# lukasvst/dm-vio

Measured on NVIDIA H100. Metric: point-residuals/sec per GN iter (7 KF, 2000 pts, 640x480), higher is better.
Workload: dtype f32

## Files before the change

### dm-vio_b200/csrc/ba_fused.cu

```cuda
#include "ba_common.cuh"
#include <cstdlib>
#include <mutex>
#include <type_traits>

namespace dmv {

template <int K, int END, class F>
__device__ __forceinline__ void static_for(F&& f) {
  if constexpr (K < END) {
    f(std::integral_constant<int, K>{});
    static_for<K + 1, END>(f);
  }
}
__host__ __device__ constexpr int top_row(int k) {
  int r = 0;
  while (r < 9 && k >= top_off(r + 1)) r++;
  return r;
}
__host__ __device__ constexpr int top_col(int k) { return top_row(k) + k - top_off(top_row(k)); }

struct PixSums {
  float JI00, JI10, JI11, JabJI00, JabJI01, JabJI10, JabJI11, Jab00, Jab01, Jab11, JIr0, JIr1, Jabr0, Jabr1, rr;
};

// ... 591 lines not shown
        const float gx = h1 * hw, gy = h2 * hw;
        const float resF = residual * hw;
        const float ja = drdA * hw, jb = hw;
        const float jaF = zA ? 0.f : ja, jbF = zB ? 0.f : jb;
        float ra = resF;
        if constexpr (MARG) { ra = (((resF - gx * jpx) - gy * jpy) - jaF * dp6) - jbF * dp7; rtz[jj] = ra; }
        sv[0] += gx * gx; sv[2] += gy * gy; sv[1] += gx * gy;
        sv[3] += ja * gx; sv[4] += ja * gy; sv[5] += jb * gx; sv[6] += jb * gy;
        sv[7] += ja * ja; sv[8] += ja * jb; sv[9] += jb * jb;
        sv[10] += ra * gx; sv[11] += ra * gy; sv[12] += ra * jaF; sv[13] += ra * jbF; sv[14] += ra * ra;
        sv[16] += hw * hw * (gx * gx + gy * gy);
      }
    }
    clk_stamp<CLK>(clk, 3, __float_as_uint(sv[0]));
    {
      const unsigned bal = __ballot_sync(0xffffffffu, fin);
      live = live && (((bal >> (lane & ~3)) & 0xfu) == 0xfu);
#pragma unroll
      for (int k = 0; k < 17; k++) {
        sv[k] += __shfl_xor_sync(0xffffffffu, sv[k], 1);
        sv[k] += __shfl_xor_sync(0xffffffffu, sv[k], 2);
      }
    }
    PixSums s = {sv[0], sv[1], sv[2], sv[3], sv[4], sv[5], sv[6], sv[7], sv[8], sv[9], sv[10], sv[11], sv[12], sv[13], sv[14]};
    const float energy = sv[15], wJI2 = sv[16];

    int newState;
    float newEnergy;
    if (st == RES_NONE) { newState = RES_NONE; newEnergy = 0.f; }
    else if (!live) { newState = RES_OOB; newEnergy = en_old; }
    else if (energy > TH || wJI2 < 2.f) { newState = RES_OUTLIER; newEnergy = TH; }
    else { newState = RES_IN; newEnergy = energy; }
    const bool in = (newState == RES_IN);
    if (st != RES_NONE && q == 0) {
      e_sum = newEnergy;
      n_in = in; n_oob = (newState == RES_OOB); n_outl = (newState == RES_OUTLIER);
    }
    if constexpr (MARG) {
      if (masked) *reinterpret_cast<float2*>(W.marg_rtz + (size_t)slot * 8 + 2 * q) = in ? make_float2(rtz[0], rtz[1]) : make_float2(0.f, 0.f);
    }
    if (valid && masked && q == 0) {
      W.st_new[slot] = (uint8_t)newState;
      W.en_new[slot] = newEnergy;
      const float ewo = (st == RES_NONE || !live) ? -1.f : energy;
      W.en_wo[slot] = ewo;
      if (t == nf - 1 && W.en_wo_newest_host) W.en_wo_newest_host[p] = ewo;
      const size_t plane = (size_t)MAXF * mp;
      W.cpt[slot] = cKu; W.cpt[plane + slot] = cKv; W.cpt[2 * plane + slot] = new_idepth;
    }

    float jp[8] = {0.f, 0.f, 0.f, 0.f, 0.f, 0.f, 0.f, 0.f}, Hdd = 0.f, bd = 0.f, Hcd0 = 0.f, Hcd1 = 0.f, Hcd2 = 0.f, Hcd3 = 0.f;
    if (in) {
      if constexpr (!MARG) geo_jac(pc, Kl0, Kl1, cu, cv, drescale, new_idepth, fx, fy, fxi, fyi, x, y, ddx, ddy);
      const float J0 = s.JI00 * ddx + s.JI10 * ddy, J1 = s.JI10 * ddx + s.JI11 * ddy;
#pragma unroll
      for (int k = 0; k < 6; k++) jp[k] = x[4 + k] * J0 + y[4 + k] * J1;
      jp[6] = s.JabJI00 * ddx + s.JabJI01 * ddy; jp[7] = s.JabJI10 * ddx + s.JabJI11 * ddy;
      Hdd = J0 * ddx + J1 * ddy;
      bd = s.JIr0 * ddx + s.JIr1 * ddy;
      Hcd0 = x[0] * J0 + y[0] * J1; Hcd1 = x[1] * J0 + y[1] * J1; Hcd2 = x[2] * J0 + y[2] * J1; Hcd3 = x[3] * J0 + y[3] * J1;
      if (valid && q == 0) {
        float4* gj = reinterpret_cast<float4*>(W.jpjd + (size_t)slot * 8);
        gj[0] = make_float4(jp[0], jp[1], jp[2], jp[3]);
        gj[1] = make_float4(jp[4], jp[5], jp[6], jp[7]);
      }
    } else {
#pragma unroll
      for (int k = 0; k < 10; k++) { x[k] = 0.f; y[k] = 0.f; }
      s = PixSums{0.f, 0.f, 0.f, 0.f, 0.f, 0.f, 0.f, 0.f, 0.f, 0.f, 0.f, 0.f, 0.f, 0.f, 0.f};
    }
    {
      const float r0 = ah[0].x * jp[0] + ah[0].y * jp[1] + ah[0].z * jp[2] + ah[0].w * jp[3] + ah[1].x * jp[4] + ah[1].y * jp[5] + ah[1].z * jp[6] + ah[1].w * jp[7];
      const float r1 = ah[2].x * jp[0] + ah[2].y * jp[1] + ah[2].z * jp[2] + ah[2].w * jp[3] + ah[3].x * jp[4] + ah[3].y * jp[5] + ah[3].z * jp[6] + ah[3].w * jp[7];
      const float j0 = (q == 0) ? jp[0] : (q == 1) ? jp[2] : (q == 2) ? jp[4] : jp[6];
      const float j1 = (q == 0) ? jp[1] : (q == 1) ? jp[3] : (q == 2) ? jp[5] : jp[7];
      if (pair_ok) {
        S.rec[t][2 * q][pl] = r0; S.rec[t][2 * q + 1][pl] = r1;
        S.Wv[pl][4 + 8 * t + 2 * q] = at2.x * j0; S.Wv[pl][4 + 8 * t + 2 * q + 1] = at2.y * j1;
      }
      const float e0 = (q == 0) ? Hdd : (q == 1) ? Hcd0 : (q == 2) ? Hcd2 : (in ? 1.f : 0.f);
      const float e1 = (q == 0) ? bd : (q == 1) ? Hcd1 : (q == 2) ? Hcd3 : 0.f;
      const int k0 = (q == 0) ? 8 : (q == 1) ? 10 : (q == 2) ? 12 : 14;
      if (pair_ok) { S.rec[t][k0][pl] = e0; S.rec[t][k0 + 1][pl] = e1; }
    }

    float v[32];
    {
      const float alq[3] = {s.JI00 * ((q == 0) ? x[0] : (q == 1) ? x[1] : (q == 2) ? x[2] : x[3]) + s.JI10 * ((q == 0) ? y[0] : (q == 1) ? y[1] : (q == 2) ? y[2] : y[3]),
                            s.JI00 * ((q == 0) ? x[4] : (q == 1) ? x[5] : (q == 2) ? x[6] : x[7]) + s.JI10 * ((q == 0) ? y[4] : (q == 1) ? y[5] : (q == 2) ? y[6] : y[7]),
                            s.JI00 * ((q == 0) ? x[8] : (q == 1) ? x[9] : 0.f) + s.JI10 * ((q == 0) ? y[8] : (q == 1) ? y[9] : 0.f)};
      const float beq[3] = {s.JI10 * ((q == 0) ? x[0] : (q == 1) ? x[1] : (q == 2) ? x[2] : x[3]) + s.JI11 * ((q == 0) ? y[0] : (q == 1) ? y[1] : (q == 2) ? y[2] : y[3]),
                            s.JI10 * ((q == 0) ? x[4] : (q == 1) ? x[5] : (q == 2) ? x[6] : x[7]) + s.JI11 * ((q == 0) ? y[4] : (q == 1) ? y[5] : (q == 2) ? y[6] : y[7]),
                            s.JI10 * ((q == 0) ? x[8] : (q == 1) ? x[9] : 0.f) + s.JI11 * ((q == 0) ? y[8] : (q == 1) ? y[9] : 0.f)};
      const float xq[3] = {(q == 0) ? x[0] : (q == 1) ? x[1] : (q == 2) ? x[2] : x[3], (q == 0) ? x[4] : (q == 1) ? x[5] : (q == 2) ? x[6] : x[7],
                           (q == 0) ? x[8] : (q == 1) ? x[9] : 0.f};
      const float yq[3] = {(q == 0) ? y[0] : (q == 1) ? y[1] : (q == 2) ? y[2] : y[3], (q == 0) ? y[4] : (q == 1) ? y[5] : (q == 2) ? y[6] : y[7],
                           (q == 0) ? y[8] : (q == 1) ? y[9] : 0.f};
      int o = 0;
#pragma unroll
      for (int j = 0; j < 3; j++) {
#pragma unroll
        for (int c = 4 * j; c < 13; c++) {
          float val;
          if (c < 10) val = alq[j] * x[c] + beq[j] * y[c];
          else if (c == 10) val = xq[j] * s.JabJI00 + yq[j] * s.JabJI01;
          else if (c == 11) val = xq[j] * s.JabJI10 + yq[j] * s.JabJI11;
          else val = xq[j] * s.JIr0 + yq[j] * s.JIr1;
          v[o++] = val;
        }
      }
      if (q == 2) { v[22] = s.Jab00; v[23] = s.Jab01; v[24] = s.Jabr0; v[25] = s.Jab11; v[26] = s.Jabr1; }
      v[27] = (q == 2) ? s.rr : 0.f;
      if (q == 3) { v[22] = v[23] = v[24] = v[25] = v[26] = 0.f; }
      v[28] = v[29] = v[30] = v[31] = 0.f;
    }
    static_for<0, 3>([&](auto sc) {
      constexpr int st2 = decltype(sc)::value, hstep = 16 >> st2, m = 16 >> st2;
      const bool up = (lane & m) != 0;
#pragma unroll
      for (int k = 0; k < hstep; k++) v[k] = (up ? v[k + hstep] : v[k]) + __shfl_xor_sync(0xffffffffu, up ? v[k] : v[k + hstep], m);
    });
    if (pair_ok) {
      const int w8 = (lane >> 2) & 7;
#pragma unroll
      for (int k = 0; k < 4; k++) {
        const int pos = 4 * w8 + k;
        int idx = -1;
        if (pos < 13) { const int rr = q, c = pos; if (c >= rr) idx = top_off(rr) + c - rr; }
        else if (pos < 22) { const int rr = q + 4, c = pos - 13 + 4; if (c >= rr) idx = top_off(rr) + c - rr; }
        else if (pos < 28) {
          if (q < 2) { const int rr = q + 8, c = pos - 22 + 8; if (pos < 27 && c >= rr) idx = top_off(rr) + c - rr; }
          else if (q == 2) idx = TOP_TRI + (pos - 22);
        }
        if (idx >= 0) S.pair[t][half][idx] = v[k];
      }
    }
  }
  }
  {
    float es = e_sum, fin = (float)n_in, foob = (float)n_oob, fout = (float)n_outl;
#pragma unroll
    for (int m = 1; m < 32; m <<= 1) {
      es += __shfl_xor_sync(0xffffffffu, es, m);
      fin += __shfl_xor_sync(0xffffffffu, fin, m);
      foob += __shfl_xor_sync(0xffffffffu, foob, m);
      fout += __shfl_xor_sync(0xffffffffu, fout, m);
      rs_step2 += __shfl_xor_sync(0xffffffffu, rs_step2, m);
      rs_nid += __shfl_xor_sync(0xffffffffu, rs_nid, m);
      rs_cnt += __shfl_xor_sync(0xffffffffu, rs_cnt, m);
    }
    if (lane == 0) {
      S.misc[warp][0] = es; S.misc[warp][1] = fin; S.misc[warp][2] = foob; S.misc[warp][3] = fout;
      S.misc[warp][4] = rs_step2; S.misc[warp][5] = rs_nid; S.misc[warp][6] = rs_cnt; S.misc[warp][7] = 0.f;
    }
  }
  cp_async_wait_all();
  __syncthreads();
  clk_stamp<CLK>(clk, 4);

  const int nt = nf - 1;
  double* __restrict__ out = W.part + (size_t)chunk * PART_STRIDE;
  {
    const int nG = nt * 26;
#pragma unroll 1
    for (int e = tid; e < nG + 9 * P + 28; e += nthreads) {
      if (e < nG) {
        const int rh = e / 13, c = e - rh * 13, i0 = (rh & 1) * 4;
        const int t = (rh >> 1) + ((rh >> 1) >= h ? 1 : 0);
        const int col = (c < 8) ? 4 + c : (c < 12 ? c - 8 : 12);
        double m[8];
#pragma unroll
        for (int k = 0; k < 8; k++) m[k] = (double)pair_entry<NH>(S.pair[t], 4 + k, col);
        const double dTc = S.dT[t][c & 7];
        const int os = (c < 8) ? 8 : (c < 12 ? 4 : 1);
        double* o = out + t * PART_SLOT + ((c < 8) ? 64 + c : (c < 12 ? 120 + c : 160)) + i0 * os;
#pragma unroll
        for (int ii = 0; ii < 4; ii++) {
          const int i = i0 + ii;
          double g = 0.0;
#pragma unroll
          for (int k = 0; k < 8; k++) g += S.AhD[t][i * 8 + k] * m[k];
          S.G[t][i][c] = g;
          double v = S.dT[t][i] * (i0 ? m[4 + ii] : m[ii]);
          if (c < 8) v = v * dTc;
          o[ii * os] = v;
        }
      } else if (e < nG + 9 * P) {
        const int k = (e - nG) / P, pl2 = (e - nG) & (P - 1);
        if (pl2 >= ch_count) continue;
        if (k < 8) {
          float sum = 0.f;
#pragma unroll
          for (int tt = 0; tt < MAXF; tt++) {
            const float v = S.rec[tt][k][pl2];
            if (tt < nf && tt != h) sum += v;
          }
          S.Wv[pl2][4 + 8 * h + k] = sum;
        } else {
          const int p = ch_start + pl2;
          float Hdd = 0.f, bd = 0.f, c0 = 0.f, c1 = 0.f, c2 = 0.f, c3 = 0.f, ngood = 0.f;
#pragma unroll 1
          for (int r = 0; r < nt; r++) {
            const int tt = r + (r >= h ? 1 : 0);
            Hdd += S.rec[tt][8][pl2]; bd += S.rec[tt][9][pl2]; c0 += S.rec[tt][10][pl2]; c1 += S.rec[tt][11][pl2];
            c2 += S.rec[tt][12][pl2]; c3 += S.rec[tt][13][pl2]; ngood += S.rec[tt][14][pl2];
          }
          float prior = S.prior[pl2];
          bool masked = true;
          if constexpr (MARG) { masked = __ldg(W.marg_mask + p) != 0; prior *= __ldg(&W.marg->priorFac); }
          float HdiF = 0.f, bdSum = 0.f, w0 = 0.f, w1 = 0.f, w2 = 0.f, w3 = 0.f;
          if (ngood > 0.f) {
            float H = Hdd + prior;
            if (H < 1e-10f) H = 1e-10f;
            HdiF = 1.0f / H;
            bdSum = MARG ? bd : bd + prior * (S.id[pl2] - S.idz[pl2]);
            w0 = c0; w1 = c1; w2 = c2; w3 = c3;
          }
          S.Wv[pl2][0] = w0; S.Wv[pl2][1] = w1; S.Wv[pl2][2] = w2; S.Wv[pl2][3] = w3;
          S.Wv[pl2][N] = bdSum;
#pragma unroll 1
          for (int c = N + 1; c < W.NW; c++) S.Wv[pl2][c] = 0.f;
          S.hdi[pl2] = HdiF;
          if (masked) {
            float4* po = reinterpret_cast<float4*>(W.pout + (size_t)p * 8);
            po[0] = make_float4(Hdd, bd, c0, c1);
            po[1] = make_float4(c2, c3, HdiF, bdSum);
          }
        }
      } else if (e < nG + 9 * P + 20) {
        const int i = (e - nG - 9 * P) / 5, j = (e - nG - 9 * P) - i * 5;
        double val = 0.0;
#pragma unroll 1
        for (int r = 0; r < nt; r++) val += (double)pair_entry<NH>(S.pair[r + (r >= h ? 1 : 0)], i, j < 4 ? j : 12);
        out[PART_CC + (j < 4 ? i * 4 + j : 16 + i)] = val;
      } else {
        const int k = e - nG - 9 * P - 20;
        double val = 0.0;
#pragma unroll 1
        for (int wv = 0; wv < nwarps; wv += 4) {
          float v[4];
#pragma unroll
          for (int u = 0; u < 4; u++) v[u] = S.misc[min(wv + u, 15)][k];
#pragma unroll
          for (int u = 0; u < 4; u++)
            if (wv + u < nwarps) val += (double)v[u];
        }
        out[PART_MISC + k] = val;
      }
    }
  }
  __syncthreads();
  {
    const int nO = nt * 16;
#pragma unroll 1
    for (int e = tid; e < 64 + nO + 8 + P * W.T; e += nthreads) {
      if (e < 64) {
        const int i = e >> 3, j = e & 7;
        double val = 0.0;
        double2 g[4], a[4];
        const int t0 = (h == 0) ? 1 : 0;
#pragma unroll
        for (int u = 0; u < 4; u++) { g[u] = reinterpret_cast<const double2*>(&S.G[t0][i][0])[u]; a[u] = reinterpret_cast<const double2*>(&S.AhD[t0][j * 8])[u]; }
#pragma unroll 1
        for (int r = 0; r < nt; r++) {
          const int tn = min(r + 1 + (r + 1 >= h ? 1 : 0), MAXF - 1);
          double2 gn[4], an[4];
#pragma unroll
          for (int u = 0; u < 4; u++) { gn[u] = reinterpret_cast<const double2*>(&S.G[tn][i][0])[u]; an[u] = reinterpret_cast<const double2*>(&S.AhD[tn][j * 8])[u]; }
#pragma unroll
          for (int u = 0; u < 4; u++) { val += g[u].x * a[u].x; val += g[u].y * a[u].y; }
#pragma unroll
          for (int u = 0; u < 4; u++) { g[u] = gn[u]; a[u] = an[u]; }
        }
        out[h * PART_SLOT + 64 + e] = val;
      } else if (e < 64 + nO) {
        const int eo = e - 64, r = eo >> 4, i = (eo >> 1) & 7, j0 = (eo & 1) * 4;
        const int t = r + (r >= h ? 1 : 0);
#pragma unroll
        for (int v = 0; v < 4; v++) out[t * PART_SLOT + i * 8 + j0 + v] = S.G[t][i][j0 + v] * S.dT[t][j0 + v];
      } else if (e < 64 + nO + 8) {
        const int i = e - 64 - nO;
        double c0 = 0.0, c1 = 0.0, c2 = 0.0, c3 = 0.0, bh = 0.0;
#pragma unroll 1
        for (int r = 0; r < nt; r++) {
          const int t2 = r + (r >= h ? 1 : 0);
          const double2 q01 = *reinterpret_cast<const double2*>(&S.G[t2][i][8]), q23 = *reinterpret_cast<const double2*>(&S.G[t2][i][10]);
          c0 += q01.x; c1 += q01.y; c2 += q23.x; c3 += q23.y; bh += S.G[t2][i][12];
        }
        double* o = out + h * PART_SLOT;
        o[128 + i * 4] = c0; o[128 + i * 4 + 1] = c1; o[128 + i * 4 + 2] = c2; o[128 + i * 4 + 3] = c3;
        o[160 + i] = bh;
      } else {
        const int ew = e - 64 - nO - 8, g4 = ew / P, pl2 = ew & (P - 1);
        if (pl2 >= ch_count) continue;
        W.wg[(size_t)g4 * mp + ch_start + pl2] = *reinterpret_cast<const float4*>(&S.Wv[pl2][4 * g4]);
        if (g4 == 0) W.hdig[ch_start + pl2] = S.hdi[pl2];
      }
    }
  }
  __syncthreads();
  clk_stamp<CLK>(clk, 5);
}

template <int P, int LPR, bool CLK = false>
__device__ __forceinline__ void fused_reduce(const BAWinDev& W, FusedSmem<P, LPR>& S, bool ok, const int vcta, const int ncta,
                                             unsigned long long* clk = nullptr) {
  const int nf = W.nf, N = W.N, mp = W.mp;
  const int tid = threadIdx.x, nthreads = blockDim.x;
  const int warp = tid >> 5, lane = tid & 31, nwarps = nthreads >> 5;

  const int nH = N * N + N;
  double* __restrict__ R = W.result;
  double* __restrict__ RH = W.result_host;
  const bool xch = W.xc.nranks > 1;
  const double* __restrict__ part = W.part;

  const int npair = nf * (nf - 1) / 2;
  const int n_off = npair * 64, n_diag = nf * 64, n_c = nf * 32, n_b = nf * 8;
  const int nitems = n_off + n_diag + n_c + n_b + 16 + 4 + (ACC_MISC - 1);
  const int grp = tid >> 4, gl = tid & 15, groups_per_cta = nthreads >> 4;
  const int nch = W.nchunks;
  const int dcta = ncta - 1 - vcta;
  auto phase_d = [&](const int pass) {
    for (int base = dcta * groups_per_cta; base < nitems; base += ncta * groups_per_cta) {
      const int item = base + grp;
      const bool act = item < nitems;
      int off0 = 0, lo0 = 0, hi0 = act ? nch : 0, off1 = 0, lo1 = 0, hi1 = 0, d0 = 0, d1 = -1;
      int e = act ? item : nitems - 1;
      if (e < n_off) {
        const int q = e >> 6, ij = e & 63, i = ij >> 3, j = ij & 7;
        int a = 0, rem = q;
        while (rem >= nf - 1 - a) { rem -= nf - 1 - a; a++; }
        const int b = a + 1 + rem;
        off0 = b * PART_SLOT + i * 8 + j; lo0 = W.chunk_beg[a]; hi0 = act ? W.chunk_beg[a + 1] : lo0;
        off1 = a * PART_SLOT + j * 8 + i; lo1 = W.chunk_beg[b]; hi1 = act ? W.chunk_beg[b + 1] : lo1;
        d0 = (4 + 8 * a + i) * N + 4 + 8 * b + j; d1 = (4 + 8 * b + j) * N + 4 + 8 * a + i;
      } else if ((e -= n_off) < n_diag) {
        const int a = e >> 6, ij = e & 63;
        off0 = a * PART_SLOT + 64 + ij;
        d0 = (4 + 8 * a + (ij >> 3)) * N + 4 + 8 * a + (ij & 7);
      } else if ((e -= n_diag) < n_c) {
        const int a = e >> 5, ic = e & 31;
        off0 = a * PART_SLOT + 128 + ic;
        d0 = (4 + 8 * a + (ic >> 2)) * N + (ic & 3); d1 = (ic & 3) * N + 4 + 8 * a + (ic >> 2);
      } else if ((e -= n_c) < n_b) {
        off0 = (e >> 3) * PART_SLOT + 160 + (e & 7);
        d0 = N * N + 4 + e;
      } else if ((e -= n_b) < 16) {
        off0 = PART_CC + e; d0 = (e >> 2) * N + (e & 3);
      } else if ((e -= 16) < 4) {
        off0 = PART_CC + 16 + e; d0 = N * N + e;
      } else {
        e -= 4;
        off0 = PART_MISC + e; d0 = nH + W.ntiles * 16 + e;
      }
      if (pass == 0) {
        double sum = 0.0;
        if (hi0 - lo0 <= 96 && hi1 - lo1 <= 96) {
          double v[12];
#pragma unroll
          for (int u = 0; u < 12; u++) {
            const int c = (u < 6 ? lo0 : lo1) + gl + 16 * (u % 6);
            v[u] = (c < (u < 6 ? hi0 : hi1)) ? __ldcg(part + (u < 6 ? off0 : off1) + (size_t)c * PART_STRIDE) : 0.0;
          }
#pragma unroll
          for (int u = 0; u < 12; u++) sum += v[u];
        } else {
#pragma unroll 1
          for (int seg = 0; seg < 2; seg++) {
            const int lo = seg ? lo1 : lo0, hi = seg ? hi1 : hi0;
            const double* __restrict__ src = part + (seg ? off1 : off0);
            for (int c0 = lo + gl; c0 < hi; c0 += 192) {
              double v[12];
#pragma unroll
              for (int u = 0; u < 12; u++) v[u] = (c0 + 16 * u < hi) ? __ldcg(src + (size_t)(c0 + 16 * u) * PART_STRIDE) : 0.0;
#pragma unroll
              for (int u = 0; u < 12; u++) sum += v[u];
            }
          }
        }
        sum += __shfl_xor_sync(0xffffffffu, sum, 8);
        sum += __shfl_xor_sync(0xffffffffu, sum, 4);
        sum += __shfl_xor_sync(0xffffffffu, sum, 2);
        sum += __shfl_xor_sync(0xffffffffu, sum, 1);
        if (gl == 0 && act) {
          if (xch) { R[d0] = sum; xchg_push(W.xc, d0, sum); }
          else { R[d0] = sum; if (d1 >= 0) R[d1] = sum; if (RH) { RH[d0] = sum; if (d1 >= 0) RH[d1] = sum; } }
        }
      } else {
        const double sum = xchg_pull_sum_group(W.xc, d0, (gl == 0 && act) ? R[d0] : 0.0, act, ok);
        if (gl == 0 && act) {
          R[d0] = sum; if (d1 >= 0) R[d1] = sum;
          if (RH) { RH[d0] = sum; if (d1 >= 0) RH[d1] = sum; }
        }
      }
    }
    };
  phase_d(0);
  clk_stamp<CLK>(clk, 7);

  {
    const int T = W.T, npts = W.npts;
    for (int tile0 = vcta; tile0 < W.ntiles; tile0 += 2 * ncta) {
      const int tile1 = tile0 + ncta;
      const bool two = tile1 < W.ntiles;
      int ti0 = 0, rem = tile0;
      while (rem >= T - ti0) { rem -= T - ti0; ti0++; }
      const int tj0 = ti0 + rem;
      int ti1 = 0;
      rem = two ? tile1 : tile0;
      while (rem >= T - ti1) { rem -= T - ti1; ti1++; }
      const int tj1 = ti1 + rem;
      float a[2][4][4];
#pragma unroll
      for (int q = 0; q < 2; q++)
#pragma unroll
        for (int i = 0; i < 4; i++)
#pragma unroll
          for (int j = 0; j < 4; j++) a[q][i][j] = 0.f;
      const float4* __restrict__ wi0 = W.wg + (size_t)ti0 * mp;
      const float4* __restrict__ wj0 = W.wg + (size_t)tj0 * mp;
      const float4* __restrict__ wi1 = W.wg + (size_t)ti1 * mp;
      const float4* __restrict__ wj1 = W.wg + (size_t)tj1 * mp;
#pragma unroll 4
      for (int p = tid; p < npts; p += nthreads) {
        const float sc = __ldcg(W.hdig + p);
        const float4 wi = __ldcg(wi0 + p), wj = __ldcg(wj0 + p);
        const float si[4] = {sc * wi.x, sc * wi.y, sc * wi.z, sc * wi.w};
        const float vj[4] = {wj.x, wj.y, wj.z, wj.w};
#pragma unroll
        for (int i = 0; i < 4; i++)
#pragma unroll
          for (int j = 0; j < 4; j++) a[0][i][j] += si[i] * vj[j];
        if (two) {
          const float4 xi = __ldcg(wi1 + p), xj = __ldcg(wj1 + p);
          const float ti[4] = {sc * xi.x, sc * xi.y, sc * xi.z, sc * xi.w};
          const float uj[4] = {xj.x, xj.y, xj.z, xj.w};
#pragma unroll
          for (int i = 0; i < 4; i++)
#pragma unroll
            for (int j = 0; j < 4; j++) a[1][i][j] += ti[i] * uj[j];
        }
      }
      {
        float d[32];
#pragma unroll
        for (int qq = 0; qq < 2; qq++)
#pragma unroll
          for (int i = 0; i < 4; i++)
#pragma unroll
            for (int j = 0; j < 4; j++) d[qq * 16 + i * 4 + j] = a[qq][i][j];
        static_for<0, 5>([&](auto sc) {
          constexpr int st2 = decltype(sc)::value, hstep = 16 >> st2, m = 16 >> st2;
          const bool up = (lane & m) != 0;
#pragma unroll
          for (int k = 0; k < hstep; k++) d[k] = (up ? d[k + hstep] : d[k]) + __shfl_xor_sync(0xffffffffu, up ? d[k] : d[k + hstep], m);
        });
        S.red[warp][lane] = (double)d[0];
      }
      __syncthreads();
      if (tid < 32) {
        const bool own = tid < 16 || two;
        double d = 0.0;
        for (int wv = 0; wv < nwarps; wv++) d += S.red[wv][tid];
        const int idx = nH + (tid < 16 ? tile0 : tile1) * 16 + (tid & 15);
        if (own) {
          R[idx] = d;
          if (xch) xchg_push(W.xc, idx, d);
          else if (RH) RH[idx] = d;
        }
      }
      __syncthreads();
    }
  }
  clk_stamp<CLK>(clk, 8);
  if (xch) {
    phase_d(1);
    if (tid < 32) {
      for (int tile0 = vcta; tile0 < W.ntiles; tile0 += 2 * ncta) {
        const int tile1 = tile0 + ncta;
        const bool own = tid < 16 || tile1 < W.ntiles;
        const int idx = nH + (tid < 16 ? tile0 : tile1) * 16 + (tid & 15);
        const double d = xchg_pull_sum_lanes(W.xc, idx, own ? R[idx] : 0.0, own, ok);
        if (own) {
          R[idx] = d;
          if (RH) RH[idx] = d;
        }
      }
    }
  }
  if (!__syncthreads_and(ok) && tid == 0) {
    R[nH + W.ntiles * 16 + 7] = 1.0;
    if (RH) RH[nH + W.ntiles * 16 + 7] = 1.0;
  }
}

template <int P> struct FusedCfgOf { static constexpr int LPR = (P == 16) ? 4 : 1, TPB = (P == 16) ? 448 : 224; };

template <int P, bool MARG, bool CLK = false>
__global__ void __launch_bounds__(FusedCfgOf<P>::TPB, 1)
    ba_fused_kernel(const __grid_constant__ BAWinDev W, const __grid_constant__ BAIter it, unsigned long long* clk) {
  constexpr int LPR = FusedCfgOf<P>::LPR;
  extern __shared__ __align__(16) unsigned char smem_raw[];
  FusedSmem<P, LPR>& S = *reinterpret_cast<FusedSmem<P, LPR>*>(smem_raw);
  clk_stamp<CLK>(clk, 0);
#pragma unroll 1
  for (int chunk = blockIdx.x; chunk < W.nchunks; chunk += gridDim.x) fused_chunk<P, LPR, MARG, CLK>(W, it, S, chunk, clk);
  const bool ok = grid_barrier(W.bar, W.bar_target);
  clk_stamp<CLK>(clk, 6);
  fused_reduce<P, LPR, CLK>(W, S, ok, blockIdx.x, gridDim.x, clk);
}

template <int P>
__global__ void __launch_bounds__(FusedCfgOf<P>::TPB, P == 32 ? 2 : 1)
    ba_fused_batch_kernel(const BAWinDev* __restrict__ gW, const BAIter* __restrict__ gIt, const __grid_constant__ BABatchHdr hdr) {
  constexpr int LPR = FusedCfgOf<P>::LPR;
  extern __shared__ __align__(16) unsigned char smem_raw[];
  FusedSmem<P, LPR>& S = *reinterpret_cast<FusedSmem<P, LPR>*>(smem_raw);
#pragma unroll 1
  for (int item = blockIdx.x; item < hdr.total; item += gridDim.x) {
    int w = 0;
    while (w + 1 < hdr.B && item >= hdr.prefix[w + 1]) w++;
    fused_chunk<P, LPR, false>(gW[w], gIt[w], S, item - hdr.prefix[w]);
  }
  const bool ok = grid_barrier(hdr.bar, hdr.bar_target);
#pragma unroll 1
  for (int w = 0; w < hdr.B; w++) fused_reduce<P, LPR>(gW[w], S, ok, (int)((blockIdx.x + (unsigned)w * 41u) % gridDim.x), gridDim.x);
}

struct FusedCfg { bool done = false; int max_ctas = 0; };
static std::mutex g_cfg_mutex;

template <int P, bool MARG, bool CLK = false>
static cudaError_t launch_cfg(BAWinDev& W, const BAIter& it, cudaStream_t s, unsigned* bar_count, unsigned long long* clk = nullptr) {
  static FusedCfg cfg[64];
  constexpr int TPB = FusedCfgOf<P>::TPB;
  int dev = 0;
  cudaError_t e = cudaGetDevice(&dev);
  if (e != cudaSuccess) return e;
  const int smem = (int)sizeof(FusedSmem<P, FusedCfgOf<P>::LPR>);
  const int threads = TPB;
  int max_ctas;
  {
    std::lock_guard<std::mutex> lk(g_cfg_mutex);
    FusedCfg& c = cfg[dev & 63];
    if (!c.done) {
      e = cudaFuncSetAttribute(ba_fused_kernel<P, MARG, CLK>, cudaFuncAttributeMaxDynamicSharedMemorySize, smem);
      if (e != cudaSuccess) return e;
      int per_sm = 0, sms = 0;
      e = cudaOccupancyMaxActiveBlocksPerMultiprocessor(&per_sm, ba_fused_kernel<P, MARG, CLK>, TPB, smem);
      if (e != cudaSuccess) return e;
      e = cudaDeviceGetAttribute(&sms, cudaDevAttrMultiProcessorCount, dev);
      if (e != cudaSuccess) return e;
      c.max_ctas = per_sm * sms;
      c.done = true;
    }
    max_ctas = c.max_ctas;
  }
  const int grid = min(W.nchunks, max_ctas);
  *bar_count += (unsigned)grid;
  W.bar_target = *bar_count;
  void* args[3] = {(void*)&W, (void*)&it, (void*)&clk};
  return cudaLaunchCooperativeKernel((const void*)ba_fused_kernel<P, MARG, CLK>, dim3(grid), dim3(threads), args, (size_t)smem, s);
}

template <int P>
static cudaError_t launch_batch_cfg(const BAWinDev* gW, const BAIter* gIt, BABatchHdr& hdr, int max_nf, cudaStream_t s, unsigned* bar_count) {
  static FusedCfg cfg[64];
  constexpr int TPB = FusedCfgOf<P>::TPB;
  int dev = 0;
  cudaError_t e = cudaGetDevice(&dev);
  if (e != cudaSuccess) return e;
  const int smem = (int)sizeof(FusedSmem<P, FusedCfgOf<P>::LPR>);
  const int threads = TPB;
  (void)max_nf;
  int max_ctas;
  {
    std::lock_guard<std::mutex> lk(g_cfg_mutex);
    FusedCfg& c = cfg[dev & 63];
    if (!c.done) {
      e = cudaFuncSetAttribute(ba_fused_batch_kernel<P>, cudaFuncAttributeMaxDynamicSharedMemorySize, smem);
      if (e != cudaSuccess) return e;
      int per_sm = 0, sms = 0;
      e = cudaOccupancyMaxActiveBlocksPerMultiprocessor(&per_sm, ba_fused_batch_kernel<P>, TPB, smem);
      if (e != cudaSuccess) return e;
      e = cudaDeviceGetAttribute(&sms, cudaDevAttrMultiProcessorCount, dev);
      if (e != cudaSuccess) return e;
      c.max_ctas = per_sm * sms;
      c.done = true;
    }
    max_ctas = c.max_ctas;
  }
  const int grid = min(hdr.total, max_ctas);
  *bar_count += (unsigned)grid;
  hdr.bar_target = *bar_count;
  void* args[3] = {(void*)&gW, (void*)&gIt, (void*)&hdr};
  return cudaLaunchCooperativeKernel((const void*)ba_fused_batch_kernel<P>, dim3(grid), dim3(threads), args, (size_t)smem, s);
}

cudaError_t launch_fused_batch_kernel(int P, const BAWinDev* gW, const BAIter* gIt, BABatchHdr& hdr, int max_nf, cudaStream_t s, unsigned* bar_count) {
  return (P == 32) ? launch_batch_cfg<32>(gW, gIt, hdr, max_nf, s, bar_count) : launch_batch_cfg<16>(gW, gIt, hdr, max_nf, s, bar_count);
}

cudaError_t launch_fused_kernel(BAWinDev& W, const BAIter& it, bool marg, cudaStream_t s, unsigned* bar_count) {
  if (W.P == 32) return marg ? launch_cfg<32, true>(W, it, s, bar_count) : launch_cfg<32, false>(W, it, s, bar_count);
  return marg ? launch_cfg<16, true>(W, it, s, bar_count) : launch_cfg<16, false>(W, it, s, bar_count);
}

cudaError_t launch_fused_kernel_clocked(BAWinDev& W, const BAIter& it, cudaStream_t s, unsigned* bar_count, unsigned long long* clk, int* grid) {
  const unsigned before = *bar_count;
  const cudaError_t e = (W.P == 32) ? launch_cfg<32, false, true>(W, it, s, bar_count, clk) : launch_cfg<16, false, true>(W, it, s, bar_count, clk);
  *grid = (int)(*bar_count - before);
  return e;
}

}
```

Baseline: 510.4 million.

## Prefetch tile-reduction loads before phase_d and pair diagonal tiles to share reads

```diff
diff --git a/dm-vio_b200/csrc/ba_fused.cu b/dm-vio_b200/csrc/ba_fused.cu
--- a/dm-vio_b200/csrc/ba_fused.cu
+++ b/dm-vio_b200/csrc/ba_fused.cu
@@ -917,7 +917,7 @@
   clk_stamp<CLK>(clk, 5);
 }
 
-template <int P, int LPR, bool CLK = false>
+template <int P, int LPR, int ED, bool CLK = false>
 __device__ __forceinline__ void fused_reduce(const BAWinDev& W, FusedSmem<P, LPR>& S, bool ok, const int vcta, const int ncta,
                                              unsigned long long* clk = nullptr) {
   const int nf = W.nf, N = W.N, mp = W.mp;
@@ -929,6 +929,44 @@
   double* __restrict__ RH = W.result_host;
   const bool xch = W.xc.nranks > 1;
   const double* __restrict__ part = W.part;
+
+  const int T = W.T, npts = W.npts;
+  const int ndiag = (T + 1) / 2, nunits = ndiag + T * (T - 1) / 2;
+  int gi = 0, gj = 0, tile0 = 0, tile1 = -1;
+  auto decode = [&](const int u) {
+    auto tile_of = [&](int i, int j) { return i * T - (i * (i - 1)) / 2 + (j - i); };
+    if (u < ndiag) {
+      gi = 2 * u; gj = min(gi + 1, T - 1);
+      tile0 = tile_of(gi, gi); tile1 = (gi + 1 < T) ? tile_of(gj, gj) : -1;
+    } else {
+      int rem = u - ndiag;
+      gi = 0;
+      while (rem >= T - 1 - gi) { rem -= T - 1 - gi; gi++; }
+      gj = gi + 1 + rem;
+      tile0 = tile_of(gi, gj); tile1 = -1;
+    }
+  };
+  const int estep = ED * nthreads;
+  float esc[ED];
+  float4 ex[ED], ey[ED];
+  auto e_load = [&](const int pb) {
+    const float4* __restrict__ wi = W.wg + (size_t)gi * mp;
+    const float4* __restrict__ wj = W.wg + (size_t)gj * mp;
+#pragma unroll
+    for (int k = 0; k < ED; k++) {
+      const int p = pb + tid + k * nthreads;
+      if (p < npts) { esc[k] = __ldcg(W.hdig + p); ex[k] = __ldcg(wi + p); ey[k] = __ldcg(wj + p); }
+    }
+  };
+  auto e_dep = [&]() {
+    unsigned d = 0u;
+    if (vcta < nunits)
+#pragma unroll
+      for (int k = 0; k < ED; k++)
+        if (tid + k * nthreads < npts) d ^= __float_as_uint(esc[k]) ^ __float_as_uint(ex[k].x) ^ __float_as_uint(ey[k].x);
+    return d;
+  };
+  bool stamped = false;
 
   const int npair = nf * (nf - 1) / 2;
   const int n_off = npair * 64, n_diag = nf * 64, n_c = nf * 32, n_b = nf * 8;
@@ -978,6 +1016,15 @@
             const int c = (u < 6 ? lo0 : lo1) + gl + 16 * (u % 6);
             v[u] = (c < (u < 6 ? hi0 : hi1)) ? __ldcg(part + (u < 6 ? off0 : off1) + (size_t)c * PART_STRIDE) : 0.0;
           }
+          if constexpr (CLK) {
+            if (!stamped) {
+              unsigned d = e_dep();
+#pragma unroll
+              for (int u = 0; u < 12; u++) d ^= (unsigned)__double_as_longlong(v[u]);
+              clk_stamp<CLK>(clk, 7, d);
+              stamped = true;
+            }
+          }
 #pragma unroll
           for (int u = 0; u < 12; u++) sum += v[u];
         } else {
@@ -1010,91 +1057,86 @@
         }
       }
     }
-    };
+  };
+
+  if (vcta < nunits) { decode(vcta); e_load(0); }
   phase_d(0);
-  clk_stamp<CLK>(clk, 7);
-
-  {
-    const int T = W.T, npts = W.npts;
-    for (int tile0 = vcta; tile0 < W.ntiles; tile0 += 2 * ncta) {
-      const int tile1 = tile0 + ncta;
-      const bool two = tile1 < W.ntiles;
-      int ti0 = 0, rem = tile0;
-      while (rem >= T - ti0) { rem -= T - ti0; ti0++; }
-      const int tj0 = ti0 + rem;
-      int ti1 = 0;
-      rem = two ? tile1 : tile0;
-      while (rem >= T - ti1) { rem -= T - ti1; ti1++; }
-      const int tj1 = ti1 + rem;
-      float a[2][4][4];
-#pragma unroll
-      for (int q = 0; q < 2; q++)
+  if constexpr (CLK) {
+    if (!stamped) clk_stamp<CLK>(clk, 7, e_dep());
+  }
+
+  for (int u = vcta; u < nunits; u += ncta) {
+    if (u != vcta) decode(u);
+    const bool diag = u < ndiag, two = tile1 >= 0;
+    float a[2][4][4];
+#pragma unroll
+    for (int q = 0; q < 2; q++)
+#pragma unroll
+      for (int i = 0; i < 4; i++)
+#pragma unroll
+        for (int j = 0; j < 4; j++) a[q][i][j] = 0.f;
+    for (int pb = 0; pb < npts; pb += estep) {
+      if (u != vcta || pb != 0) e_load(pb);
+#pragma unroll
+      for (int k = 0; k < ED; k++) {
+        if (pb + tid + k * nthreads < npts) {
+          const float sc = esc[k];
+          const float4 wi = ex[k], wj = diag ? ex[k] : ey[k];
+          const float si[4] = {sc * wi.x, sc * wi.y, sc * wi.z, sc * wi.w};
+          const float vj[4] = {wj.x, wj.y, wj.z, wj.w};
+#pragma unroll
+          for (int i = 0; i < 4; i++)
+#pragma unroll
+            for (int j = 0; j < 4; j++) a[0][i][j] += si[i] * vj[j];
+          if (two) {
+            const float4 xj = ey[k];
+            const float ti[4] = {sc * xj.x, sc * xj.y, sc * xj.z, sc * xj.w};
+            const float uj[4] = {xj.x, xj.y, xj.z, xj.w};
+#pragma unroll
+            for (int i = 0; i < 4; i++)
+#pragma unroll
+              for (int j = 0; j < 4; j++) a[1][i][j] += ti[i] * uj[j];
+          }
+        }
+      }
+    }
+    {
+      float d[32];
+#pragma unroll
+      for (int qq = 0; qq < 2; qq++)
 #pragma unroll
         for (int i = 0; i < 4; i++)
 #pragma unroll
-          for (int j = 0; j < 4; j++) a[q][i][j] = 0.f;
-      const float4* __restrict__ wi0 = W.wg + (size_t)ti0 * mp;
-      const float4* __restrict__ wj0 = W.wg + (size_t)tj0 * mp;
-      const float4* __restrict__ wi1 = W.wg + (size_t)ti1 * mp;
-      const float4* __restrict__ wj1 = W.wg + (size_t)tj1 * mp;
-#pragma unroll 4
-      for (int p = tid; p < npts; p += nthreads) {
-        const float sc = __ldcg(W.hdig + p);
-        const float4 wi = __ldcg(wi0 + p), wj = __ldcg(wj0 + p);
-        const float si[4] = {sc * wi.x, sc * wi.y, sc * wi.z, sc * wi.w};
-        const float vj[4] = {wj.x, wj.y, wj.z, wj.w};
-#pragma unroll
-        for (int i = 0; i < 4; i++)
-#pragma unroll
-          for (int j = 0; j < 4; j++) a[0][i][j] += si[i] * vj[j];
-        if (two) {
-          const float4 xi = __ldcg(wi1 + p), xj = __ldcg(wj1 + p);
-          const float ti[4] = {sc * xi.x, sc * xi.y, sc * xi.z, sc * xi.w};
-          const float uj[4] = {xj.x, xj.y, xj.z, xj.w};
-#pragma unroll
-          for (int i = 0; i < 4; i++)
-#pragma unroll
-            for (int j = 0; j < 4; j++) a[1][i][j] += ti[i] * uj[j];
-        }
-      }
-      {
-        float d[32];
-#pragma unroll
-        for (int qq = 0; qq < 2; qq++)
-#pragma unroll
-          for (int i = 0; i < 4; i++)
-#pragma unroll
-            for (int j = 0; j < 4; j++) d[qq * 16 + i * 4 + j] = a[qq][i][j];
-        static_for<0, 5>([&](auto sc) {
-          constexpr int st2 = decltype(sc)::value, hstep = 16 >> st2, m = 16 >> st2;
-          const bool up = (lane & m) != 0;
-#pragma unroll
-          for (int k = 0; k < hstep; k++) d[k] = (up ? d[k + hstep] : d[k]) + __shfl_xor_sync(0xffffffffu, up ? d[k] : d[k + hstep], m);
-        });
-        S.red[warp][lane] = (double)d[0];
-      }
-      __syncthreads();
-      if (tid < 32) {
-        const bool own = tid < 16 || two;
-        double d = 0.0;
-        for (int wv = 0; wv < nwarps; wv++) d += S.red[wv][tid];
-        const int idx = nH + (tid < 16 ? tile0 : tile1) * 16 + (tid & 15);
-        if (own) {
-          R[idx] = d;
-          if (xch) xchg_push(W.xc, idx, d);
-          else if (RH) RH[idx] = d;
-        }
-      }
-      __syncthreads();
-    }
+          for (int j = 0; j < 4; j++) d[qq * 16 + i * 4 + j] = a[qq][i][j];
+      static_for<0, 5>([&](auto sc) {
+        constexpr int st2 = decltype(sc)::value, hstep = 16 >> st2, m = 16 >> st2;
+        const bool up = (lane & m) != 0;
+#pragma unroll
+        for (int k = 0; k < hstep; k++) d[k] = (up ? d[k + hstep] : d[k]) + __shfl_xor_sync(0xffffffffu, up ? d[k] : d[k + hstep], m);
+      });
+      S.red[warp][lane] = (double)d[0];
+    }
+    __syncthreads();
+    if (tid < 32) {
+      const bool own = tid < 16 || two;
+      double d = 0.0;
+      for (int wv = 0; wv < nwarps; wv++) d += S.red[wv][tid];
+      const int idx = nH + (tid < 16 ? tile0 : tile1) * 16 + (tid & 15);
+      if (own) {
+        R[idx] = d;
+        if (xch) xchg_push(W.xc, idx, d);
+        else if (RH) RH[idx] = d;
+      }
+    }
+    __syncthreads();
   }
   clk_stamp<CLK>(clk, 8);
   if (xch) {
     phase_d(1);
     if (tid < 32) {
-      for (int tile0 = vcta; tile0 < W.ntiles; tile0 += 2 * ncta) {
-        const int tile1 = tile0 + ncta;
-        const bool own = tid < 16 || tile1 < W.ntiles;
+      for (int u = vcta; u < nunits; u += ncta) {
+        decode(u);
+        const bool own = tid < 16 || tile1 >= 0;
         const int idx = nH + (tid < 16 ? tile0 : tile1) * 16 + (tid & 15);
         const double d = xchg_pull_sum_lanes(W.xc, idx, own ? R[idx] : 0.0, own, ok);
         if (own) {
@@ -1110,7 +1152,7 @@
   }
 }
 
-template <int P> struct FusedCfgOf { static constexpr int LPR = (P == 16) ? 4 : 1, TPB = (P == 16) ? 448 : 224; };
+template <int P> struct FusedCfgOf { static constexpr int LPR = (P == 16) ? 4 : 1, TPB = (P == 16) ? 448 : 224, ED = 2240 / TPB; };
 
 template <int P, bool MARG, bool CLK = false>
 __global__ void __launch_bounds__(FusedCfgOf<P>::TPB, 1)
@@ -1123,7 +1165,7 @@
   for (int chunk = blockIdx.x; chunk < W.nchunks; chunk += gridDim.x) fused_chunk<P, LPR, MARG, CLK>(W, it, S, chunk, clk);
   const bool ok = grid_barrier(W.bar, W.bar_target);
   clk_stamp<CLK>(clk, 6);
-  fused_reduce<P, LPR, CLK>(W, S, ok, blockIdx.x, gridDim.x, clk);
+  fused_reduce<P, LPR, FusedCfgOf<P>::ED, CLK>(W, S, ok, blockIdx.x, gridDim.x, clk);
 }
 
 template <int P>
@@ -1140,7 +1182,7 @@
   }
   const bool ok = grid_barrier(hdr.bar, hdr.bar_target);
 #pragma unroll 1
-  for (int w = 0; w < hdr.B; w++) fused_reduce<P, LPR>(gW[w], S, ok, (int)((blockIdx.x + (unsigned)w * 41u) % gridDim.x), gridDim.x);
+  for (int w = 0; w < hdr.B; w++) fused_reduce<P, LPR, 5>(gW[w], S, ok, (int)((blockIdx.x + (unsigned)w * 41u) % gridDim.x), gridDim.x);
 }
 
 struct FusedCfg { bool done = false; int max_ctas = 0; };
```

Measured after the change: 519.1 million, median of 6. +1.7%, better.
